# olivier-2018/scene_3Dreconstruction_MVSNet

Measured on AMD Instinct MI355X. Metric: depth maps/sec at N=5 views, 640x512, D=192; achieved HBM GB/s, higher is better.
Workload: dtype f32 (conv0, conv2-4, conv9, conv11: 3xbf16 split operands on the bf16 matrix cores, fp32 accumulate)

## Files before the change

scene_3dreconstruction_mvsnet_amd/csrc/conv0_split.hip:

```cpp
#include <cstring>
#include <type_traits>

#include "mvs_internal.h"
#include "storage.h"

namespace mvs {

typedef unsigned int su32x4 __attribute__((ext_vector_type(4)));
typedef unsigned int su32x2 __attribute__((ext_vector_type(2)));
typedef __bf16 sbf16x8 __attribute__((ext_vector_type(8)));

__device__ __forceinline__ f32x4 mfma_bf16(su32x4 a, su32x4 b, f32x4 c) {
    return __builtin_amdgcn_mfma_f32_16x16x32_bf16(__builtin_bit_cast(sbf16x8, a), __builtin_bit_cast(sbf16x8, b), c, 0, 0, 0);
}

namespace c48t {
constexpr int TZ = 4, TY = 8, TX = 32;
constexpr int HY = TY + 2, HX = TX + 2;
constexpr int NT_PLANES = 6, NPL = 3;
constexpr int VOX = HY * HX;
constexpr int PLANE_E = VOX * 8;
constexpr int PIECE_E = NPL * PLANE_E;
constexpr int BUF_E = 3 * PIECE_E;
constexpr int NCOL = VOX * 2;
constexpr int CPT = (NCOL + 255) / 256;
constexpr int NPOS = TY * TX;
constexpr int EXS = 8;
constexpr int MAXT = 512;
static_assert(2 * BUF_E * 2 + NT_PLANES * NPOS * EXS * 4 + MAXT * 16 <= 160 * 1024, "LDS of conv0_w48t");
constexpr unsigned bstep(int s) { return (unsigned)(((s >> 1) * NT_PLANES + 3 * (s & 1)) * 9) * 1024u; }
__device__ __forceinline__ int chunk_of(int k, int c) { return (k & 1) ? 3 - c : c; }
__device__ __forceinline__ unsigned bofs(int chunk, int h) { return (unsigned)((chunk * NT_PLANES + 3 * h) * 9) * 1024u; }
}
typedef float sf32x2 __attribute__((ext_vector_type(2)));
typedef __bf16 sbf16x2 __attribute__((ext_vector_type(2)));

__device__ __forceinline__ sf32x2 split_stage(const sf32x2 a, unsigned& packed) {
    const sbf16x2 h = __builtin_convertvector(a, sbf16x2);
    packed = __builtin_bit_cast(unsigned, h);
    const sf32x2 w = {__uint_as_float(packed << 16), __uint_as_float(packed & 0xFFFF0000u)};
    return a - w;
}
__device__ __forceinline__ void split3x(const f32x4 v, su32x2& p1, su32x2& p2, su32x2& p3) {
    unsigned a0, a1, b0, b1, c0, c1;
    const sf32x2 r0 = split_stage((sf32x2){v.x, v.y}, a0), r1 = split_stage((sf32x2){v.z, v.w}, a1);
    const sf32x2 q0 = split_stage(r0, b0), q1 = split_stage(r1, b1);
    c0 = __builtin_bit_cast(unsigned, __builtin_convertvector(q0, sbf16x2));
    c1 = __builtin_bit_cast(unsigned, __builtin_convertvector(q1, sbf16x2));
    p1 = (su32x2){a0, a1};
    p2 = (su32x2){b0, b1};
    p3 = (su32x2){c0, c1};
}

__device__ __forceinline__ void c48t_step_mfmas(const unsigned short* __restrict__ tile, const int (&aoff)[3],
                                                const su32x4 (&B)[2][3][3], su32x4 (&Bn)[2][3][3],
                                                __amdgpu_buffer_rsrc_t brs, const unsigned (&bvoff)[2], unsigned bnext,
                                                f32x4 (&acc)[3][2]) {
    using namespace c48t;
    constexpr int NC = 9;
    su32x4 a[3][4];
    auto request = [&](int n) {
        const int pn = n / 3, in = n % 3;
#pragma unroll
        for (int j = 0; j < 4; ++j)
            a[n % 3][j] = *reinterpret_cast<const su32x4*>(tile + pn * PIECE_E + aoff[in] + j * HX * 8);
    };
    request(0);
    request(1);
#pragma unroll
    for (int n = 0; n < NC; ++n) {
        const int p = n / 3, i = n % 3;
        if (n + 2 < NC) request(n + 2);
#pragma unroll
        for (int f = 2 * n; f < 2 * n + 2; ++f)
            Bn[f / 9][(f / 3) % 3][f % 3] = __builtin_bit_cast(su32x4, __builtin_amdgcn_raw_buffer_load_b128(
                brs, (int)bvoff[f / 9], (int)(bnext + (unsigned)(f % 9) * 1024u), 0));
        const int pl = i == 2 ? 1 : 0;
#pragma unroll
        for (int ky = 0; ky < 3; ++ky)
#pragma unroll
            for (int q = 0; q < 3 - p; ++q)
#pragma unroll
                for (int rr = 0; rr < 2; ++rr)
                    acc[i][rr] = mfma_bf16(a[n % 3][rr + ky], B[pl][ky][q], acc[i][rr]);
        __builtin_amdgcn_sched_barrier(0);
    }
}

__global__ __launch_bounds__(512) void conv0_w48t_kernel(
    const float* __restrict__ x,
    const unsigned short* __restrict__ bp,
    const float* __restrict__ bias,
    float* __restrict__ y,
    int D, int H, int W, int nb
    ) {
    using namespace c48t;
    __shared__ __attribute__((aligned(16))) unsigned short buf[2 * BUF_E];
    __shared__ __attribute__((aligned(16))) float ex[NT_PLANES * NPOS * EXS];
    __shared__ int org[MAXT][4];

    const int tid = threadIdx.x, lane = tid & 63, wave = tid >> 6;
    const bool consumer = __builtin_amdgcn_readfirstlane(wave) < 4;
    const int nbx = (W + TX - 1) / TX, nby = (H + TY - 1) / TY;
    const int G = gridDim.x;
    const int ntile = (nb - (int)blockIdx.x + G - 1) / G;
    const size_t HW8 = (size_t)H * W * 8, V8 = (size_t)D * HW8;
    auto origin = [&](int idx, int& x0, int& y0, int& z0) {
        int bx, by, bz;
        if (nby % 8 == 0 && G % 8 == 0) {
            const int xcd = idx & 7, rows = nby >> 3;
            int i = idx >> 3;
            bx = i % nbx; i /= nbx;
            by = xcd * rows + i % rows;
            bz = i / rows;
        } else {
            int b = idx;
            bx = b % nbx; b /= nbx;
            by = b % nby;
            bz = b / nby;
        }
        x0 = bx * TX; y0 = by * TY; z0 = bz * TZ;
    };

    for (int j = tid; j < ntile; j += 512) {
        int x0, y0, z0;
        origin((int)blockIdx.x + j * G, x0, y0, z0);
        org[j][0] = x0; org[j][1] = y0; org[j][2] = z0;
    }
    __syncthreads();
    const int ptid = tid & 255;

    if (consumer) {
        const int r = lane & 15, g = lane >> 4, cw = wave;
        const int pa = (0x2100 >> (4 * cw)) & 15, ra = (0x1220 >> (4 * cw)) & 15;
        const int pb = (0x2211 >> (4 * cw)) & 15, rb = (0x3010 >> (4 * cw)) & 15;
        const int upl[3] = {pa, pa, pb}, urp[3] = {ra, ra + 1, rb};
        int aoff[3];
#pragma unroll
        for (int i = 0; i < 3; ++i) aoff[i] = upl[i] * PLANE_E + ((2 * urp[i]) * HX + 2 * r + g) * 8;
        su32x4 B[2][2][3][3];
        const __amdgpu_buffer_rsrc_t brs = __builtin_amdgcn_make_buffer_rsrc(
            const_cast<unsigned short*>(bp), (short)0, 4 * NT_PLANES * 9 * 1024, 0x00020000);
        const unsigned bvoff[2] = {(unsigned)lane * 16u + (unsigned)pa * 9u * 1024u,
                                   (unsigned)lane * 16u + (unsigned)pb * 9u * 1024u};
#pragma unroll
        for (int f = 0; f < 18; ++f)
            B[0][f / 9][(f / 3) % 3][f % 3] = __builtin_bit_cast(su32x4, __builtin_amdgcn_raw_buffer_load_b128(
                brs, (int)bvoff[f / 9], (int)(bstep(0) + (unsigned)(f % 9) * 1024u), 0));
        f32x4 acc[2][3][2];
#pragma unroll
        for (int h = 0; h < 2; ++h)
#pragma unroll
            for (int i = 0; i < 3; ++i)
#pragma unroll
                for (int n = 0; n < 2; ++n) acc[h][i][n] = (f32x4){0.f, 0.f, 0.f, 0.f};
        auto exchange = [&]() {
            const int n = lane & 15, jj = n >> 3, co = n & 7;
#pragma unroll
            for (int h = 0; h < 2; ++h)
#pragma unroll
                for (int i = 0; i < 3; ++i)
#pragma unroll
                    for (int rr = 0; rr < 2; ++rr)
#pragma unroll
                        for (int e = 0; e < 4; ++e) {
                            ex[((3 * h + upl[i]) * NPOS + (2 * urp[i] + rr) * TX + 2 * (4 * g + e) + jj) * EXS + co] = acc[h][i][rr][e];
                            acc[h][i][rr][e] = 0.0f;
                        }
        };
        const __amdgpu_buffer_rsrc_t yrs = __builtin_amdgcn_make_buffer_rsrc(y, (short)0, (int)(V8 * 4), 0x00020000);
        const f32x4 obias = *reinterpret_cast<const f32x4*>(bias + (ptid & 1) * 4);
        auto output = [&](int j, int it, bool live) {
            const int x0 = org[j][0], y0 = org[j][1], z0 = org[j][2];
            const int pos = (ptid >> 1) + it * (NPOS / 2), ch = ptid & 1;
            const int gy = y0 + (pos >> 5), gx = x0 + (pos & 31);
            const bool ok = live && gy < H && gx < W;
            f32x4 M[NT_PLANES];
#pragma unroll
            for (int q = 0; q < NT_PLANES; ++q) M[q] = *reinterpret_cast<const f32x4*>(ex + (q * NPOS + pos) * EXS + ch * 4);
            const f32x4 zero = (f32x4){0.f, 0.f, 0.f, 0.f};
            const f32x4 s12 = M[1] + M[2], d12 = M[1] - M[2], s34 = M[3] + M[4], d34 = M[3] - M[4];
            f32x4 o[TZ];
            o[0] = (M[0] + s12) + s34;
            o[1] = d12 + 2.0f * d34;
            o[2] = s12 + 4.0f * s34;
            o[3] = (d12 + 8.0f * d34) + M[5];
            const unsigned base = (unsigned)((((size_t)z0 * H + gy) * W + gx) * 8 + ch * 4) * 4u;
#pragma unroll
            for (int q = 0; q < TZ; ++q) {
                const f32x4 v = __builtin_elementwise_max(o[q] + obias, zero);
                const unsigned off = (ok && z0 + q < D) ? base + (unsigned)q * (unsigned)(HW8 * 4) : 0xFFFFFFF0u;
                __builtin_amdgcn_raw_buffer_store_b128(__builtin_bit_cast(su32x4, v), yrs, (int)off, 0, 0);
            }
        };
        int kk = 0;
        auto cstep = [&](auto s_tag) {
            constexpr int s = decltype(s_tag)::value, h = s & 1;
            if (s == 1 || s == 3) output(kk > 0 ? kk - 1 : 0, s >> 1, kk > 0);
            c48t_step_mfmas(buf + h * BUF_E, aoff, B[h], B[h ^ 1], brs, bvoff,
                            s < 7 ? bofs(chunk_of(kk, (s + 1) >> 1), (s + 1) & 1) : bofs(chunk_of(kk + 1, 0), 0), acc[h]);
            if (s == 7) exchange();
        };
        __syncthreads();
#pragma unroll 1
        for (int k = 0; k < ntile; ++k) {
            kk = k;
            cstep(std::integral_constant<int, 0>{});
            __syncthreads();
            cstep(std::integral_constant<int, 1>{});
            __syncthreads();
            cstep(std::integral_constant<int, 2>{});
            __syncthreads();
            cstep(std::integral_constant<int, 3>{});
            __syncthreads();
            cstep(std::integral_constant<int, 4>{});
            __syncthreads();
            cstep(std::integral_constant<int, 5>{});
            __syncthreads();
            cstep(std::integral_constant<int, 6>{});
            __syncthreads();
            cstep(std::integral_constant<int, 7>{});
            __syncthreads();
        }
        output(ntile - 1, 0, true);
        output(ntile - 1, 1, true);
    } else {
        __builtin_amdgcn_s_setprio(2);
        unsigned boff[CPT][NT_PLANES];
        int loff[CPT];
        int chy[CPT], chx[CPT], crel[CPT];
#pragma unroll
        for (int i = 0; i < CPT; ++i) {
            const int col = min(ptid + i * 256, NCOL - 1);
            loff[i] = col;
            const int half = col & 1, v = col >> 1;
            chx[i] = v % HX - 1;
            chy[i] = v / HX - 1;
            crel[i] = (chy[i] * W + chx[i]) * 8 + half * 4;
        }
        auto set_tile = [&](int j) {
            const int x0 = org[j][0], y0 = org[j][1], z0 = org[j][2];
            const int hw8 = (int)HW8, tbase = (y0 * W + x0) * 8;
#pragma unroll
            for (int i = 0; i < CPT; ++i) {
                const int gy = y0 + chy[i], gx = x0 + chx[i];
                const bool ok = (unsigned)gy < (unsigned)H && (unsigned)gx < (unsigned)W;
                const int cb = tbase + crel[i];
#pragma unroll
                for (int q = 0; q < NT_PLANES; ++q) {
                    const int gz = z0 - 1 + q;
                    boff[i][q] = (ok && (unsigned)gz < (unsigned)D) ? (unsigned)(gz * hw8 + cb) * 4u
                                                                      : 0x80000000u;
                }
            }
        };
        auto rsrc = [&](int c) {
            return __builtin_amdgcn_make_buffer_rsrc(const_cast<float*>(x + (size_t)c * V8), (short)0, (int)(V8 * 4), 0x00020000);
        };
        f32x4 stg[CPT][NT_PLANES];
        f32x4 hold[CPT][NPL];
        auto put = [&](unsigned short* dstbuf, int i, int t, const f32x4 u) {
            su32x2 p1, p2, p3;
            split3x(u, p1, p2, p3);
            su32x2* dst = reinterpret_cast<su32x2*>(dstbuf) + t * (PLANE_E / 4) + loff[i];
            dst[0] = p1;
            dst[PIECE_E / 4] = p2;
            dst[2 * (PIECE_E / 4)] = p3;
        };
        auto process0 = [&](int cn) {
            const __amdgpu_buffer_rsrc_t rs = rsrc(cn);
#pragma unroll
            for (int i = 0; i < CPT; ++i) {
                f32x4 d[NT_PLANES];
#pragma unroll
                for (int q = 0; q < NT_PLANES; ++q) d[q] = stg[i][q];
                const f32x4 t1 = d[4] - 4.0f * d[2], t2 = d[3] - 4.0f * d[1];
                const f32x4 t3 = d[4] - d[2], t4 = 2.0f * (d[3] - d[1]);
                const f32x4 u0 = 4.0f * d[0] - 5.0f * d[2] + d[4];
                const f32x4 u1 = t1 + t2, u2 = t1 - t2;
                hold[i][0] = t3 + t4;
                hold[i][1] = t3 - t4;
                hold[i][2] = 4.0f * d[1] - 5.0f * d[3] + d[5];
                const f32x4 u[NPL] = {u0, u1, u2};
#pragma unroll
                for (int t = 0; t < NPL; ++t) {
#pragma unroll
                    for (int q = 2 * t; q < 2 * t + 2; ++q)
                        stg[i][q] = __builtin_bit_cast(f32x4, __builtin_amdgcn_raw_buffer_load_b128(rs, (int)boff[i][q], 0, 0));
                    put(buf, i, t, u[t]);
                    __builtin_amdgcn_sched_barrier(0);
                }
            }
        };
        auto process1 = [&]() {
#pragma unroll
            for (int i = 0; i < CPT; ++i)
#pragma unroll
                for (int t = 0; t < NPL; ++t) {
                    put(buf + BUF_E, i, t, hold[i][t]);
                    __builtin_amdgcn_sched_barrier(0);
                }
        };
        auto pstep = [&](int k, auto s_tag) {
            constexpr int s = decltype(s_tag)::value, c = s >> 1, h = s & 1;
            if (s == 5 && k + 1 < ntile) set_tile(k + 1);
            if (h == 0) process1();
            else process0(c < 2 ? chunk_of(k, c + 2) : chunk_of(k + 1, c - 2));
        };
        set_tile(0);
        {
            const __amdgpu_buffer_rsrc_t rs = rsrc(0);
#pragma unroll
            for (int i = 0; i < CPT; ++i)
#pragma unroll
                for (int q = 0; q < NT_PLANES; ++q)
                    stg[i][q] = __builtin_bit_cast(f32x4, __builtin_amdgcn_raw_buffer_load_b128(rs, (int)boff[i][q], 0, 0));
        }
        process0(1);
        __syncthreads();
#pragma unroll 1
        for (int k = 0; k < ntile; ++k) {
            pstep(k, std::integral_constant<int, 0>{});
            __syncthreads();
            pstep(k, std::integral_constant<int, 1>{});
            __syncthreads();
            pstep(k, std::integral_constant<int, 2>{});
            __syncthreads();
            pstep(k, std::integral_constant<int, 3>{});
            __syncthreads();
            pstep(k, std::integral_constant<int, 4>{});
            __syncthreads();
            pstep(k, std::integral_constant<int, 5>{});
            __syncthreads();
            pstep(k, std::integral_constant<int, 6>{});
            __syncthreads();
            pstep(k, std::integral_constant<int, 7>{});
            __syncthreads();
        }
    }
}

int launch_conv0_wino43_split(const void* x, void* y, const void* bp, const float* bias, int D, int H, int W,
                              int dtype, hipStream_t s) {
    using namespace c48t;
    if (dtype != MVS_F32) return fail(MVS_ERR_BAD_DTYPE, "conv0_wino43_split: fp32 volumes only (dtype %d)", dtype);
    if ((size_t)D * H * W * 8 * 4 >= ((size_t)1 << 31))
        return fail(MVS_ERR_BAD_SHAPE, "conv0_wino43_split: plane of %zu bytes exceeds 31-bit buffer offsets",
                    (size_t)D * H * W * 8 * 4);
    const int nb = ((W + TX - 1) / TX) * ((H + TY - 1) / TY) * ((D + TZ - 1) / TZ);
    const int cus = device_cus();
    int grid = nb < cus ? nb : cus;
    if ((nb + grid - 1) / grid > MAXT) grid = (nb + MAXT - 1) / MAXT;
    conv0_w48t_kernel<<<grid, 512, 0, s>>>(static_cast<const float*>(x), static_cast<const unsigned short*>(bp), bias,
                                           static_cast<float*>(y), D, H, W, nb);
    return check_hip(hipGetLastError(), "conv0_w48t launch");
}

static inline uint16_t bf16_rne(float v) {
    uint32_t u;
    std::memcpy(&u, &v, 4);
    if ((u & 0x7F800000u) == 0x7F800000u && (u & 0x007FFFFFu)) return (uint16_t)((u >> 16) | 0x0040u);
    u += 0x7FFFu + ((u >> 16) & 1u);
    return (uint16_t)(u >> 16);
}
static inline float bf16_to_f32(uint16_t h) {
    const uint32_t u = (uint32_t)h << 16;
    float v;
    std::memcpy(&v, &u, 4);
    return v;
}

void pack_conv0_wino43_split_weights(const float* wfold, void* out) {
    uint16_t* bp = static_cast<uint16_t*>(out);
    for (int c = 0; c < 4; ++c)
        for (int t = 0; t < 6; ++t)
            for (int ky = 0; ky < 3; ++ky)
                for (int lane = 0; lane < 64; ++lane)
                    for (int j = 0; j < 8; ++j) {
                        const int n = lane & 15, g = lane >> 4, jj = n >> 3, co = n & 7, kx = g - jj;
                        float gv = 0.0f;
                        if (kx >= 0 && kx <= 2) {
                            const int tap = ky * 3 + kx, ci = 8 * c + j;
                            const double g0 = wfold[((size_t)(0 * 9 + tap) * 32 + ci) * 8 + co];
                            const double g1 = wfold[((size_t)(1 * 9 + tap) * 32 + ci) * 8 + co];
                            const double g2 = wfold[((size_t)(2 * 9 + tap) * 32 + ci) * 8 + co];
                            double gd;
                            switch (t) {
                                case 0: gd = g0 / 4.0; break;
                                case 1: gd = -(g0 + g1 + g2) / 6.0; break;
                                case 2: gd = -(g0 - g1 + g2) / 6.0; break;
                                case 3: gd = g0 / 24.0 + g1 / 12.0 + g2 / 6.0; break;
                                case 4: gd = g0 / 24.0 - g1 / 12.0 + g2 / 6.0; break;
                                default: gd = g2; break;
                            }
                            gv = (float)gd;
                        }
                        const uint16_t h1 = bf16_rne(gv);
                        const float r1 = gv - bf16_to_f32(h1);
                        const uint16_t h2 = bf16_rne(r1);
                        const float r2 = r1 - bf16_to_f32(h2);
                        const uint16_t h3 = bf16_rne(r2);
                        const uint16_t hs[3] = {h1, h2, h3};
                        for (int q = 0; q < 3; ++q)
                            bp[((((size_t)(c * 6 + t) * 3 + ky) * 3 + q) * 64 + lane) * 8 + j] = hs[q];
                    }
}

}
```

Baseline: 1546.

## Restructure conv0 Winograd kernel: 8 producer waves, LDS-staged weights, in-register output transform

Changes the warp-specialized conv0 kernel from 4 producer waves to 8 (768 threads), so each producer handles fewer columns. Weight fragments are no longer loaded straight from global memory into registers. Consumer waves copy them into double-buffered LDS with buffer_load_lds and read them back per step. Each consumer wave now owns whole rows across all six Winograd planes, so the inverse transform, bias and ReLU run from accumulators in registers. This removes the LDS exchange buffer and its extra pass, at the cost of scalar 4-byte stores instead of 16-byte ones and more register pressure from holding all A fragments.

```diff
diff --git a/scene_3dreconstruction_mvsnet_amd/csrc/conv0_split.hip b/scene_3dreconstruction_mvsnet_amd/csrc/conv0_split.hip
--- a/scene_3dreconstruction_mvsnet_amd/csrc/conv0_split.hip
+++ b/scene_3dreconstruction_mvsnet_amd/csrc/conv0_split.hip
@@ -14,7 +14,7 @@
     return __builtin_amdgcn_mfma_f32_16x16x32_bf16(__builtin_bit_cast(sbf16x8, a), __builtin_bit_cast(sbf16x8, b), c, 0, 0, 0);
 }
 
-namespace c48t {
+namespace c12 {
 constexpr int TZ = 4, TY = 8, TX = 32;
 constexpr int HY = TY + 2, HX = TX + 2;
 constexpr int NT_PLANES = 6, NPL = 3;
@@ -23,12 +23,12 @@
 constexpr int PIECE_E = NPL * PLANE_E;
 constexpr int BUF_E = 3 * PIECE_E;
 constexpr int NCOL = VOX * 2;
-constexpr int CPT = (NCOL + 255) / 256;
-constexpr int NPOS = TY * TX;
-constexpr int EXS = 8;
+constexpr int NCW = 4, NPW = 8;
+constexpr int NFR = NPL * 9;
+constexpr int BBUF_E = NFR * 512;
+constexpr int FPW = (NFR + NCW - 1) / NCW;
 constexpr int MAXT = 512;
-static_assert(2 * BUF_E * 2 + NT_PLANES * NPOS * EXS * 4 + MAXT * 16 <= 160 * 1024, "LDS of conv0_w48t");
-constexpr unsigned bstep(int s) { return (unsigned)(((s >> 1) * NT_PLANES + 3 * (s & 1)) * 9) * 1024u; }
+static_assert(2 * BUF_E * 2 + 2 * BBUF_E * 2 + MAXT * 16 <= 160 * 1024, "LDS of conv0_w12");
 __device__ __forceinline__ int chunk_of(int k, int c) { return (k & 1) ? 3 - c : c; }
 __device__ __forceinline__ unsigned bofs(int chunk, int h) { return (unsigned)((chunk * NT_PLANES + 3 * h) * 9) * 1024u; }
 }
@@ -52,55 +52,193 @@
     p3 = (su32x2){c0, c1};
 }
 
-__device__ __forceinline__ void c48t_step_mfmas(const unsigned short* __restrict__ tile, const int (&aoff)[3],
-                                                const su32x4 (&B)[2][3][3], su32x4 (&Bn)[2][3][3],
-                                                __amdgpu_buffer_rsrc_t brs, const unsigned (&bvoff)[2], unsigned bnext,
-                                                f32x4 (&acc)[3][2]) {
-    using namespace c48t;
-    constexpr int NC = 9;
-    su32x4 a[3][4];
-    auto request = [&](int n) {
-        const int pn = n / 3, in = n % 3;
-#pragma unroll
-        for (int j = 0; j < 4; ++j)
-            a[n % 3][j] = *reinterpret_cast<const su32x4*>(tile + pn * PIECE_E + aoff[in] + j * HX * 8);
-    };
-    request(0);
-    request(1);
-#pragma unroll
-    for (int n = 0; n < NC; ++n) {
-        const int p = n / 3, i = n % 3;
-        if (n + 2 < NC) request(n + 2);
-#pragma unroll
-        for (int f = 2 * n; f < 2 * n + 2; ++f)
-            Bn[f / 9][(f / 3) % 3][f % 3] = __builtin_bit_cast(su32x4, __builtin_amdgcn_raw_buffer_load_b128(
-                brs, (int)bvoff[f / 9], (int)(bnext + (unsigned)(f % 9) * 1024u), 0));
-        const int pl = i == 2 ? 1 : 0;
-#pragma unroll
-        for (int ky = 0; ky < 3; ++ky)
-#pragma unroll
-            for (int q = 0; q < 3 - p; ++q)
-#pragma unroll
-                for (int rr = 0; rr < 2; ++rr)
-                    acc[i][rr] = mfma_bf16(a[n % 3][rr + ky], B[pl][ky][q], acc[i][rr]);
+template <typename Pre, typename Copy>
+__device__ __forceinline__ void c12_step_mfmas(const unsigned short* __restrict__ tile, const unsigned short* __restrict__ bt,
+                                               int aoff, int boff, f32x4 (&acc)[3][2], Pre&& pre, Copy&& copy) {
+    using namespace c12;
+    constexpr int NG = 27, DB = 4;
+    su32x4 a[3][3][4], b[NG];
+    auto ra = [&](int i, int p, int j) {
+        a[i][p][j] = *reinterpret_cast<const su32x4*>(tile + i * PLANE_E + p * PIECE_E + aoff + j * HX * 8);
+    };
+    auto rb = [&](int n) {
+        const int i = n / 9, q = (n / 3) % 3, ky = n % 3;
+        b[n] = *reinterpret_cast<const su32x4*>(bt + ((i * 3 + ky) * 3 + q) * 512 + boff);
+    };
+    rb(0);
+    ra(0, 0, 0);
+    ra(0, 0, 1);
+    __builtin_amdgcn_sched_barrier(0);
+#pragma unroll
+    for (int p = 1; p < 3; ++p) {
+        ra(0, p, 0);
+        ra(0, p, 1);
+    }
+    __builtin_amdgcn_sched_barrier(0);
+#pragma unroll
+    for (int n = 1; n < DB; ++n) rb(n);
+#pragma unroll
+    for (int p = 0; p < 3; ++p) {
+        ra(0, p, 2);
+        ra(0, p, 3);
+    }
+    pre();
+    __builtin_amdgcn_sched_barrier(0);
+#pragma unroll
+    for (int n = 0; n < NG; ++n) {
+        const int i = n / 9, k = n % 9, q = k / 3, ky = k % 3;
+        if (n + DB < NG) rb(n + DB);
+        if (i + 1 < 3) {
+            if (k == 0) { ra(i + 1, 0, 0); ra(i + 1, 0, 1); ra(i + 1, 0, 2); ra(i + 1, 0, 3); }
+            if (k == 1) ra(i + 1, 1, 0);
+            if (k == 2) ra(i + 1, 1, 1);
+            if (k == 3) { ra(i + 1, 1, 2); ra(i + 1, 1, 3); }
+            if (k == 4) ra(i + 1, 2, 0);
+            if (k == 5) ra(i + 1, 2, 1);
+            if (k == 6) { ra(i + 1, 2, 2); ra(i + 1, 2, 3); }
+        }
+        if (n >= 1 && n <= FPW) copy(n - 1);
+#pragma unroll
+        for (int p = 0; p < 3 - q; ++p)
+#pragma unroll
+            for (int rr = 0; rr < 2; ++rr) acc[i][rr] = mfma_bf16(a[i][p][rr + ky], b[n], acc[i][rr]);
         __builtin_amdgcn_sched_barrier(0);
     }
 }
 
-__global__ __launch_bounds__(512) void conv0_w48t_kernel(
+template <int NP>
+__device__ __forceinline__ void c12_produce(const float* __restrict__ x, unsigned short* __restrict__ buf,
+                                            const int (*__restrict__ org)[4], int D, int H, int W, int ntile, int pw,
+                                            int lane) {
+    using namespace c12;
+    const size_t HW8 = (size_t)H * W * 8, V8 = (size_t)D * HW8;
+    unsigned boff[NP][NT_PLANES];
+    int loff[NP];
+    int chy[NP], chx[NP], crel[NP];
+#pragma unroll
+    for (int i = 0; i < NP; ++i) {
+        const int col = min(pw * 64 + lane + i * NPW * 64, NCOL - 1);
+        loff[i] = col;
+        const int half = col & 1, v = col >> 1;
+        chx[i] = v % HX - 1;
+        chy[i] = v / HX - 1;
+        crel[i] = (chy[i] * W + chx[i]) * 8 + half * 4;
+    }
+    auto set_tile = [&](int j) {
+        const int x0 = org[j][0], y0 = org[j][1], z0 = org[j][2];
+        const int hw8 = (int)HW8, tbase = (y0 * W + x0) * 8;
+#pragma unroll
+        for (int i = 0; i < NP; ++i) {
+            const int gy = y0 + chy[i], gx = x0 + chx[i];
+            const bool ok = (unsigned)gy < (unsigned)H && (unsigned)gx < (unsigned)W;
+            const int cb = tbase + crel[i];
+#pragma unroll
+            for (int q = 0; q < NT_PLANES; ++q) {
+                const int gz = z0 - 1 + q;
+                boff[i][q] = (ok && (unsigned)gz < (unsigned)D) ? (unsigned)(gz * hw8 + cb) * 4u
+                                                                  : 0x80000000u;
+            }
+        }
+    };
+    auto rsrc = [&](int c) {
+        return __builtin_amdgcn_make_buffer_rsrc(const_cast<float*>(x + (size_t)c * V8), (short)0, (int)(V8 * 4), 0x00020000);
+    };
+    f32x4 stg[NP][NT_PLANES];
+    f32x4 hold[NP][NPL];
+    auto put = [&](unsigned short* dstbuf, int i, int t, const f32x4 u) {
+        su32x2 p1, p2, p3;
+        split3x(u, p1, p2, p3);
+        su32x2* dst = reinterpret_cast<su32x2*>(dstbuf) + t * (PLANE_E / 4) + loff[i];
+        dst[0] = p1;
+        dst[PIECE_E / 4] = p2;
+        dst[2 * (PIECE_E / 4)] = p3;
+    };
+    auto process0 = [&](int cn) {
+        const __amdgpu_buffer_rsrc_t rs = rsrc(cn);
+#pragma unroll
+        for (int i = 0; i < NP; ++i) {
+            f32x4 d[NT_PLANES];
+#pragma unroll
+            for (int q = 0; q < NT_PLANES; ++q) d[q] = stg[i][q];
+            const f32x4 t1 = d[4] - 4.0f * d[2], t2 = d[3] - 4.0f * d[1];
+            const f32x4 t3 = d[4] - d[2], t4 = 2.0f * (d[3] - d[1]);
+            const f32x4 u0 = 4.0f * d[0] - 5.0f * d[2] + d[4];
+            const f32x4 u1 = t1 + t2, u2 = t1 - t2;
+            hold[i][0] = t3 + t4;
+            hold[i][1] = t3 - t4;
+            hold[i][2] = 4.0f * d[1] - 5.0f * d[3] + d[5];
+            const f32x4 u[NPL] = {u0, u1, u2};
+#pragma unroll
+            for (int t = 0; t < NPL; ++t) {
+#pragma unroll
+                for (int q = 2 * t; q < 2 * t + 2; ++q)
+                    stg[i][q] = __builtin_bit_cast(f32x4, __builtin_amdgcn_raw_buffer_load_b128(rs, (int)boff[i][q], 0, 0));
+                put(buf, i, t, u[t]);
+                __builtin_amdgcn_sched_barrier(0);
+            }
+        }
+    };
+    auto process1 = [&]() {
+#pragma unroll
+        for (int i = 0; i < NP; ++i)
+#pragma unroll
+            for (int t = 0; t < NPL; ++t) {
+                put(buf + BUF_E, i, t, hold[i][t]);
+                __builtin_amdgcn_sched_barrier(0);
+            }
+    };
+    auto pstep = [&](int k, auto s_tag) {
+        constexpr int s = decltype(s_tag)::value, c = s >> 1, h = s & 1;
+        if (s == 5 && k + 1 < ntile) set_tile(k + 1);
+        if (h == 0) process1();
+        else process0(c < 2 ? chunk_of(k, c + 2) : chunk_of(k + 1, c - 2));
+    };
+    set_tile(0);
+    {
+        const __amdgpu_buffer_rsrc_t rs = rsrc(0);
+#pragma unroll
+        for (int i = 0; i < NP; ++i)
+#pragma unroll
+            for (int q = 0; q < NT_PLANES; ++q)
+                stg[i][q] = __builtin_bit_cast(f32x4, __builtin_amdgcn_raw_buffer_load_b128(rs, (int)boff[i][q], 0, 0));
+    }
+    process0(1);
+    __syncthreads();
+#pragma unroll 1
+    for (int k = 0; k < ntile; ++k) {
+        pstep(k, std::integral_constant<int, 0>{});
+        __syncthreads();
+        pstep(k, std::integral_constant<int, 1>{});
+        __syncthreads();
+        pstep(k, std::integral_constant<int, 2>{});
+        __syncthreads();
+        pstep(k, std::integral_constant<int, 3>{});
+        __syncthreads();
+        pstep(k, std::integral_constant<int, 4>{});
+        __syncthreads();
+        pstep(k, std::integral_constant<int, 5>{});
+        __syncthreads();
+        pstep(k, std::integral_constant<int, 6>{});
+        __syncthreads();
+        pstep(k, std::integral_constant<int, 7>{});
+        __syncthreads();
+    }
+}
+
+__global__ __launch_bounds__(768) void conv0_w12_kernel(
     const float* __restrict__ x,
     const unsigned short* __restrict__ bp,
     const float* __restrict__ bias,
     float* __restrict__ y,
     int D, int H, int W, int nb
     ) {
-    using namespace c48t;
+    using namespace c12;
     __shared__ __attribute__((aligned(16))) unsigned short buf[2 * BUF_E];
-    __shared__ __attribute__((aligned(16))) float ex[NT_PLANES * NPOS * EXS];
+    __shared__ __attribute__((aligned(16))) unsigned short bb0[BBUF_E], bb1[BBUF_E];
     __shared__ int org[MAXT][4];
 
-    const int tid = threadIdx.x, lane = tid & 63, wave = tid >> 6;
-    const bool consumer = __builtin_amdgcn_readfirstlane(wave) < 4;
+    const int tid = threadIdx.x, lane = tid & 63;
+    const int wave = __builtin_amdgcn_readfirstlane(tid >> 6);
     const int nbx = (W + TX - 1) / TX, nby = (H + TY - 1) / TY;
     const int G = gridDim.x;
     const int ntile = (nb - (int)blockIdx.x + G - 1) / G;
@@ -122,31 +260,23 @@
         x0 = bx * TX; y0 = by * TY; z0 = bz * TZ;
     };
 
-    for (int j = tid; j < ntile; j += 512) {
+    for (int j = tid; j < ntile; j += 768) {
         int x0, y0, z0;
         origin((int)blockIdx.x + j * G, x0, y0, z0);
         org[j][0] = x0; org[j][1] = y0; org[j][2] = z0;
     }
     __syncthreads();
-    const int ptid = tid & 255;
-
-    if (consumer) {
+
+    if (wave < NCW) {
         const int r = lane & 15, g = lane >> 4, cw = wave;
-        const int pa = (0x2100 >> (4 * cw)) & 15, ra = (0x1220 >> (4 * cw)) & 15;
-        const int pb = (0x2211 >> (4 * cw)) & 15, rb = (0x3010 >> (4 * cw)) & 15;
-        const int upl[3] = {pa, pa, pb}, urp[3] = {ra, ra + 1, rb};
-        int aoff[3];
-#pragma unroll
-        for (int i = 0; i < 3; ++i) aoff[i] = upl[i] * PLANE_E + ((2 * urp[i]) * HX + 2 * r + g) * 8;
-        su32x4 B[2][2][3][3];
+        const int aoff = ((2 * cw) * HX + 2 * r + g) * 8;
         const __amdgpu_buffer_rsrc_t brs = __builtin_amdgcn_make_buffer_rsrc(
             const_cast<unsigned short*>(bp), (short)0, 4 * NT_PLANES * 9 * 1024, 0x00020000);
-        const unsigned bvoff[2] = {(unsigned)lane * 16u + (unsigned)pa * 9u * 1024u,
-                                   (unsigned)lane * 16u + (unsigned)pb * 9u * 1024u};
-#pragma unroll
-        for (int f = 0; f < 18; ++f)
-            B[0][f / 9][(f / 3) % 3][f % 3] = __builtin_bit_cast(su32x4, __builtin_amdgcn_raw_buffer_load_b128(
-                brs, (int)bvoff[f / 9], (int)(bstep(0) + (unsigned)(f % 9) * 1024u), 0));
+        auto copy_b = [&](unsigned short* dst, unsigned src, int j) {
+            const int f = min(cw * FPW + j, NFR - 1);
+            __builtin_amdgcn_raw_ptr_buffer_load_lds(brs, (__attribute__((address_space(3))) void*)(dst + f * 512), 16,
+                                                     lane * 16, (int)(src + (unsigned)f * 1024u), 0, 0);
+        };
         f32x4 acc[2][3][2];
 #pragma unroll
         for (int h = 0; h < 2; ++h)
@@ -154,53 +284,51 @@
             for (int i = 0; i < 3; ++i)
 #pragma unroll
                 for (int n = 0; n < 2; ++n) acc[h][i][n] = (f32x4){0.f, 0.f, 0.f, 0.f};
-        auto exchange = [&]() {
-            const int n = lane & 15, jj = n >> 3, co = n & 7;
-#pragma unroll
-            for (int h = 0; h < 2; ++h)
-#pragma unroll
-                for (int i = 0; i < 3; ++i)
-#pragma unroll
-                    for (int rr = 0; rr < 2; ++rr)
-#pragma unroll
-                        for (int e = 0; e < 4; ++e) {
-                            ex[((3 * h + upl[i]) * NPOS + (2 * urp[i] + rr) * TX + 2 * (4 * g + e) + jj) * EXS + co] = acc[h][i][rr][e];
-                            acc[h][i][rr][e] = 0.0f;
-                        }
-        };
         const __amdgpu_buffer_rsrc_t yrs = __builtin_amdgcn_make_buffer_rsrc(y, (short)0, (int)(V8 * 4), 0x00020000);
-        const f32x4 obias = *reinterpret_cast<const f32x4*>(bias + (ptid & 1) * 4);
-        auto output = [&](int j, int it, bool live) {
+        const int jj = r >> 3, co = r & 7;
+        const float obias = bias[co];
+        auto output = [&](int j, bool live) {
             const int x0 = org[j][0], y0 = org[j][1], z0 = org[j][2];
-            const int pos = (ptid >> 1) + it * (NPOS / 2), ch = ptid & 1;
-            const int gy = y0 + (pos >> 5), gx = x0 + (pos & 31);
-            const bool ok = live && gy < H && gx < W;
-            f32x4 M[NT_PLANES];
-#pragma unroll
-            for (int q = 0; q < NT_PLANES; ++q) M[q] = *reinterpret_cast<const f32x4*>(ex + (q * NPOS + pos) * EXS + ch * 4);
-            const f32x4 zero = (f32x4){0.f, 0.f, 0.f, 0.f};
-            const f32x4 s12 = M[1] + M[2], d12 = M[1] - M[2], s34 = M[3] + M[4], d34 = M[3] - M[4];
-            f32x4 o[TZ];
-            o[0] = (M[0] + s12) + s34;
-            o[1] = d12 + 2.0f * d34;
-            o[2] = s12 + 4.0f * s34;
-            o[3] = (d12 + 8.0f * d34) + M[5];
-            const unsigned base = (unsigned)((((size_t)z0 * H + gy) * W + gx) * 8 + ch * 4) * 4u;
-#pragma unroll
-            for (int q = 0; q < TZ; ++q) {
-                const f32x4 v = __builtin_elementwise_max(o[q] + obias, zero);
-                const unsigned off = (ok && z0 + q < D) ? base + (unsigned)q * (unsigned)(HW8 * 4) : 0xFFFFFFF0u;
-                __builtin_amdgcn_raw_buffer_store_b128(__builtin_bit_cast(su32x4, v), yrs, (int)off, 0, 0);
-            }
+#pragma unroll
+            for (int rr = 0; rr < 2; ++rr)
+#pragma unroll
+                for (int e = 0; e < 4; ++e) {
+                    const int gy = y0 + 2 * cw + rr, gx = x0 + 2 * (4 * g + e) + jj;
+                    const bool ok = live && gy < H && gx < W;
+                    float M[NT_PLANES];
+#pragma unroll
+                    for (int t = 0; t < NT_PLANES; ++t) {
+                        M[t] = acc[t / 3][t % 3][rr][e];
+                        acc[t / 3][t % 3][rr][e] = 0.0f;
+                    }
+                    const float s12 = M[1] + M[2], d12 = M[1] - M[2], s34 = M[3] + M[4], d34 = M[3] - M[4];
+                    float o[TZ];
+                    o[0] = (M[0] + s12) + s34;
+                    o[1] = d12 + 2.0f * d34;
+                    o[2] = s12 + 4.0f * s34;
+                    o[3] = (d12 + 8.0f * d34) + M[5];
+                    const unsigned base = (unsigned)((((size_t)z0 * H + gy) * W + gx) * 8 + co) * 4u;
+#pragma unroll
+                    for (int q = 0; q < TZ; ++q) {
+                        const float v = fmaxf(o[q] + obias, 0.0f);
+                        const unsigned off = (ok && z0 + q < D) ? base + (unsigned)q * (unsigned)(HW8 * 4) : 0xFFFFFFF0u;
+                        __builtin_amdgcn_raw_buffer_store_b32(__float_as_uint(v), yrs, (int)off, 0, 0);
+                    }
+                }
         };
         int kk = 0;
         auto cstep = [&](auto s_tag) {
             constexpr int s = decltype(s_tag)::value, h = s & 1;
-            if (s == 1 || s == 3) output(kk > 0 ? kk - 1 : 0, s >> 1, kk > 0);
-            c48t_step_mfmas(buf + h * BUF_E, aoff, B[h], B[h ^ 1], brs, bvoff,
-                            s < 7 ? bofs(chunk_of(kk, (s + 1) >> 1), (s + 1) & 1) : bofs(chunk_of(kk + 1, 0), 0), acc[h]);
-            if (s == 7) exchange();
+            const unsigned bnext = s < 7 ? bofs(chunk_of(kk, (s + 1) >> 1), (s + 1) & 1) : bofs(chunk_of(kk + 1, 0), 0);
+            c12_step_mfmas(
+                buf + h * BUF_E, h ? bb1 : bb0, aoff, lane * 8, acc[h],
+                [&]() { if (s == 0) output(kk > 0 ? kk - 1 : 0, kk > 0); },
+                [&](int j) { copy_b(h ? bb0 : bb1, bnext, j); });
+            __builtin_amdgcn_s_waitcnt(0x0F70);
         };
+#pragma unroll
+        for (int j = 0; j < FPW; ++j) copy_b(bb0, bofs(chunk_of(0, 0), 0), j);
+        __builtin_amdgcn_s_waitcnt(0x0F70);
         __syncthreads();
 #pragma unroll 1
         for (int k = 0; k < ntile; ++k) {
@@ -222,127 +350,18 @@
             cstep(std::integral_constant<int, 7>{});
             __syncthreads();
         }
-        output(ntile - 1, 0, true);
-        output(ntile - 1, 1, true);
+        output(ntile - 1, true);
     } else {
+        const int pw = wave - NCW;
         __builtin_amdgcn_s_setprio(2);
-        unsigned boff[CPT][NT_PLANES];
-        int loff[CPT];
-        int chy[CPT], chx[CPT], crel[CPT];
-#pragma unroll
-        for (int i = 0; i < CPT; ++i) {
-            const int col = min(ptid + i * 256, NCOL - 1);
-            loff[i] = col;
-            const int half = col & 1, v = col >> 1;
-            chx[i] = v % HX - 1;
-            chy[i] = v / HX - 1;
-            crel[i] = (chy[i] * W + chx[i]) * 8 + half * 4;
-        }
-        auto set_tile = [&](int j) {
-            const int x0 = org[j][0], y0 = org[j][1], z0 = org[j][2];
-            const int hw8 = (int)HW8, tbase = (y0 * W + x0) * 8;
-#pragma unroll
-            for (int i = 0; i < CPT; ++i) {
-                const int gy = y0 + chy[i], gx = x0 + chx[i];
-                const bool ok = (unsigned)gy < (unsigned)H && (unsigned)gx < (unsigned)W;
-                const int cb = tbase + crel[i];
-#pragma unroll
-                for (int q = 0; q < NT_PLANES; ++q) {
-                    const int gz = z0 - 1 + q;
-                    boff[i][q] = (ok && (unsigned)gz < (unsigned)D) ? (unsigned)(gz * hw8 + cb) * 4u
-                                                                      : 0x80000000u;
-                }
-            }
-        };
-        auto rsrc = [&](int c) {
-            return __builtin_amdgcn_make_buffer_rsrc(const_cast<float*>(x + (size_t)c * V8), (short)0, (int)(V8 * 4), 0x00020000);
-        };
-        f32x4 stg[CPT][NT_PLANES];
-        f32x4 hold[CPT][NPL];
-        auto put = [&](unsigned short* dstbuf, int i, int t, const f32x4 u) {
-            su32x2 p1, p2, p3;
-            split3x(u, p1, p2, p3);
-            su32x2* dst = reinterpret_cast<su32x2*>(dstbuf) + t * (PLANE_E / 4) + loff[i];
-            dst[0] = p1;
-            dst[PIECE_E / 4] = p2;
-            dst[2 * (PIECE_E / 4)] = p3;
-        };
-        auto process0 = [&](int cn) {
-            const __amdgpu_buffer_rsrc_t rs = rsrc(cn);
-#pragma unroll
-            for (int i = 0; i < CPT; ++i) {
-                f32x4 d[NT_PLANES];
-#pragma unroll
-                for (int q = 0; q < NT_PLANES; ++q) d[q] = stg[i][q];
-                const f32x4 t1 = d[4] - 4.0f * d[2], t2 = d[3] - 4.0f * d[1];
-                const f32x4 t3 = d[4] - d[2], t4 = 2.0f * (d[3] - d[1]);
-                const f32x4 u0 = 4.0f * d[0] - 5.0f * d[2] + d[4];
-                const f32x4 u1 = t1 + t2, u2 = t1 - t2;
-                hold[i][0] = t3 + t4;
-                hold[i][1] = t3 - t4;
-                hold[i][2] = 4.0f * d[1] - 5.0f * d[3] + d[5];
-                const f32x4 u[NPL] = {u0, u1, u2};
-#pragma unroll
-                for (int t = 0; t < NPL; ++t) {
-#pragma unroll
-                    for (int q = 2 * t; q < 2 * t + 2; ++q)
-                        stg[i][q] = __builtin_bit_cast(f32x4, __builtin_amdgcn_raw_buffer_load_b128(rs, (int)boff[i][q], 0, 0));
-                    put(buf, i, t, u[t]);
-                    __builtin_amdgcn_sched_barrier(0);
-                }
-            }
-        };
-        auto process1 = [&]() {
-#pragma unroll
-            for (int i = 0; i < CPT; ++i)
-#pragma unroll
-                for (int t = 0; t < NPL; ++t) {
-                    put(buf + BUF_E, i, t, hold[i][t]);
-                    __builtin_amdgcn_sched_barrier(0);
-                }
-        };
-        auto pstep = [&](int k, auto s_tag) {
-            constexpr int s = decltype(s_tag)::value, c = s >> 1, h = s & 1;
-            if (s == 5 && k + 1 < ntile) set_tile(k + 1);
-            if (h == 0) process1();
-            else process0(c < 2 ? chunk_of(k, c + 2) : chunk_of(k + 1, c - 2));
-        };
-        set_tile(0);
-        {
-            const __amdgpu_buffer_rsrc_t rs = rsrc(0);
-#pragma unroll
-            for (int i = 0; i < CPT; ++i)
-#pragma unroll
-                for (int q = 0; q < NT_PLANES; ++q)
-                    stg[i][q] = __builtin_bit_cast(f32x4, __builtin_amdgcn_raw_buffer_load_b128(rs, (int)boff[i][q], 0, 0));
-        }
-        process0(1);
-        __syncthreads();
-#pragma unroll 1
-        for (int k = 0; k < ntile; ++k) {
-            pstep(k, std::integral_constant<int, 0>{});
-            __syncthreads();
-            pstep(k, std::integral_constant<int, 1>{});
-            __syncthreads();
-            pstep(k, std::integral_constant<int, 2>{});
-            __syncthreads();
-            pstep(k, std::integral_constant<int, 3>{});
-            __syncthreads();
-            pstep(k, std::integral_constant<int, 4>{});
-            __syncthreads();
-            pstep(k, std::integral_constant<int, 5>{});
-            __syncthreads();
-            pstep(k, std::integral_constant<int, 6>{});
-            __syncthreads();
-            pstep(k, std::integral_constant<int, 7>{});
-            __syncthreads();
-        }
+        if (pw * 64 + NPW * 64 < NCOL) c12_produce<2>(x, buf, org, D, H, W, ntile, pw, lane);
+        else c12_produce<1>(x, buf, org, D, H, W, ntile, pw, lane);
     }
 }
 
 int launch_conv0_wino43_split(const void* x, void* y, const void* bp, const float* bias, int D, int H, int W,
                               int dtype, hipStream_t s) {
-    using namespace c48t;
+    using namespace c12;
     if (dtype != MVS_F32) return fail(MVS_ERR_BAD_DTYPE, "conv0_wino43_split: fp32 volumes only (dtype %d)", dtype);
     if ((size_t)D * H * W * 8 * 4 >= ((size_t)1 << 31))
         return fail(MVS_ERR_BAD_SHAPE, "conv0_wino43_split: plane of %zu bytes exceeds 31-bit buffer offsets",
@@ -351,9 +370,9 @@
     const int cus = device_cus();
     int grid = nb < cus ? nb : cus;
     if ((nb + grid - 1) / grid > MAXT) grid = (nb + MAXT - 1) / MAXT;
-    conv0_w48t_kernel<<<grid, 512, 0, s>>>(static_cast<const float*>(x), static_cast<const unsigned short*>(bp), bias,
-                                           static_cast<float*>(y), D, H, W, nb);
-    return check_hip(hipGetLastError(), "conv0_w48t launch");
+    conv0_w12_kernel<<<grid, 768, 0, s>>>(static_cast<const float*>(x), static_cast<const unsigned short*>(bp), bias,
+                                          static_cast<float*>(y), D, H, W, nb);
+    return check_hip(hipGetLastError(), "conv0_w12 launch");
 }
 
 static inline uint16_t bf16_rne(float v) {
```

After: 1555, median of 6. About the same (+0.6%).
